# bfloat16/latent-diffusion-speech

Hardware: AMD Instinct MI355X
Metric: mel_frames_per_sec (higher is better)
Workload: dtype f32; 1 GPU; configs[1]: batch=16x512-frame utterances per GPU, 50-step dpm-solver, unet1d denoiser, 80-ch mel; pipeline=sampler, utterances_per_gpu=16, frames=512, nfe=50, method=dpm-solver, parallelism=batch-shard x1

## Files before the change

### latent-diffusion-speech_amd/csrc/kernels.h

```cpp
#pragma once
#include <hip/hip_runtime.h>
#include <stddef.h>
#include <stdint.h>

#include <atomic>
#include <string>

namespace lds {

enum { ACT_NONE = 0, ACT_LRELU = 2 };
enum { EPI_NONE = 0, EPI_GEGLU = 1, EPI_TANH = 2, EPI_GELU = 3, EPI_SWISH = 4, EPI_GLU = 5 };

struct ConvArgs {
    const float* x1; const float* x2;
    int C1, C2;
    int Tsrc;
    int Tin;
    long long xb1, xb2;
    const float* w;
    int Mp, Co, Ci, KT, stride, dil, pad, ups;
    int act_in; float slope;
    const float* bias;
    const float* bias_bc;
    const float* res;
// ... 19 lines not shown

struct ConvDownArgs {
    const float* x; const float* w; const float* bias; float* out;
    int Ci, Co, K, stride, pad, L, To, B;
    float slope;
    int tile;
    const int* vlen_in; const int* vlen;
};
hipError_t launch_conv_down(const ConvDownArgs& a, hipStream_t s);
const char* conv_down_last_config();
hipError_t launch_vae_head(const float* y, const float* noise, float* out, float* z, int B, int C, int T, int only_mean, hipStream_t s,
                           const int* tlen = nullptr);

struct VocPairArgs {
    const float* x; float* out;
    const float* w1; const float* b1; int Mp1;
    const float* w2; const float* b2; int Mp2;
    int C, KT, dil, B, T;
    int accum; float out_div; float slope;
    const int* vlen;
};
bool voc_pair_applies(int C, int KT, int dil);
hipError_t launch_voc_pair(const VocPairArgs& a, hipStream_t s);
const char* voc_pair_last_config();

size_t packed_conv_elems(int Co, int Ci, int K, int* Mp_out);

struct DmaConvArgs {
    const float* x1; const float* x2;
    int C1, C2, Tsrc;
    const float* w;
    const float* bias;
    int Mp, Co, Ci, KT, stride, pad, ups;
    const float* res;
    int epi;
    float* out;
    int out_plain;
    int plain_from; float* out2;
    int vt_D;
    float2* lnpart_out;
    float2* gnpart_out;
    const float2* ln_part; int ln_np; float ln_eps; const float* ln_c1; const float* ln_c2;
    const float2* gnf_part; int gnf_groups; float gnf_eps; const float* gnf_cg; const float* gnf_c2;
    int Cout, To, B;
    int voc;
    int dil;
    int xpad, opad;
    float act_slope;
    float* out_act;
    const float* acc_in;
    float out_div;
    int ph_log2, ph_tpad, ph_Tout, ph_Cout;
    int out_f32;
    float acc_scale;
    int tile_batch;
    const int* lens; int lvl_in, lvl_out;
    const int* vlen;
    int ksplit;
    float* kpart; unsigned* kcount;
    long long kpart_cap; int kcount_cap;
    unsigned ord_m[3], ord_s;
};
struct DmaMagic { unsigned m, s; };
inline DmaMagic dma_magic(unsigned d) {
    unsigned s = 0;
    while ((1ull << s) < d) ++s;
    return DmaMagic{(unsigned)((1ull << (31 + s)) / d + 1), s};
}
__host__ __device__ inline unsigned dma_magic_div(unsigned n, unsigned m, unsigned s) {
    return (unsigned)(((unsigned long long)(n << 1) * m) >> 32) >> s;
}
struct DmaTile { int mb, nb, b, ksp; };
inline DmaTile dma_tile_of(int id, int total, int nMb, int nN, int S, const unsigned* ord_m, unsigned ord_s) {
    const int xcd = id & 7, slot = id >> 3, per = total >> 3, rem = total & 7;
    const unsigned L = (unsigned)(xcd * per + (xcd < rem ? xcd : rem) + slot);
    const unsigned tb = dma_magic_div(L, ord_m[0], ord_s & 255);
    const unsigned by = dma_magic_div(tb, ord_m[1], (ord_s >> 8) & 255);
    const unsigned b = dma_magic_div(by, ord_m[2], (ord_s >> 16) & 255);
    return DmaTile{(int)(L - tb * nMb), (int)(tb - by * nN), (int)b, (int)(by - b * S)};
}
hipError_t launch_conv_dma(const DmaConvArgs& a, int cfg, hipStream_t s);
hipError_t launch_conv_dma_pair(const DmaConvArgs& a3, const DmaConvArgs& a1, hipStream_t s);
bool conv_dma_pair_applies(const DmaConvArgs& a3, const DmaConvArgs& a1);
const char* conv_dma_last_config();

hipError_t launch_conv_bf3(const DmaConvArgs& a, int cfg, int nprod, int fmt, hipStream_t s);
hipError_t launch_conv_bf3_pair(const DmaConvArgs& a3, const DmaConvArgs& a1, int fmt, hipStream_t s);
bool conv_bf3_pair_applies(const DmaConvArgs& a3, const DmaConvArgs& a1);
const char* conv_bf3_last_config();
void conv_bf3_set_debug_rule(int r);
hipError_t launch_to_k8b3(const float* in, void* out, int B, int C, int T, int Ctot, int c_off, hipStream_t s, int fmt = 0, const int* lens = nullptr);
hipError_t launch_from_k8b3(const void* in, float* out, int B, int C, int T, hipStream_t s, int fmt = 0);
hipError_t launch_gn_stream_bf3(const void* x1, const void* x2, int C1, int C2, int T, int groups, float eps, const float* gamma,
                                const float* beta, const float* scale_shift, int ss_stride, int ss_off, int silu, const float2* gp1,
                                const float2* gp2, void* y, int B, hipStream_t s, int fmt = 0, const int* lens = nullptr, int lvl = 0);
hipError_t launch_gn_partials_bf3(const void* x, int C, int T, float2* gp, int B, hipStream_t s, int fmt = 0);
hipError_t launch_resample_k8b3(const void* in, void* out, int B, int C, int Tin, int Tout, hipStream_t s, int fmt = 0, const int* lens = nullptr, int lvl_in = 0, int lvl_out = 0);

hipError_t launch_to_k4p(const float* in, float* out, int B, int C, int T, int Ctot, int c_off, hipStream_t s, const int* lens = nullptr);
hipError_t launch_from_k4p(const float* in, float* out, int B, int C, int T, hipStream_t s);
hipError_t launch_from_k4p_pad(const float* in, float* out, int B, int C, int T, int pad, hipStream_t s);
hipError_t launch_plain_to_vt(const float* in, float* out, int B, int C, int T, int D, hipStream_t s);
hipError_t launch_gn_stream(const float* x1, const float* x2, int C1, int C2, int T, int groups, float eps,
                            const float* gamma, const float* beta, const float* scale_shift, int ss_stride, int ss_off,
                            int silu, const float2* gp1, const float2* gp2, float* y, int B, hipStream_t s, const int* lens = nullptr, int lvl = 0);
hipError_t launch_gn_partials(const float* x, int C, int T, float2* gp, int B, hipStream_t s);
hipError_t launch_to_k4p_act(const float* in, float* raw, float* act, float slope, int B, int C, int T, int pad, hipStream_t s, const int* vlen = nullptr);
hipError_t launch_k4p_zero_pads(float* x, int B, int C, int T, int pad, hipStream_t s);
hipError_t launch_resample_k4p(const float* in, float* out, int B, int C, int Tin, int Tout, hipStream_t s, const int* lens = nullptr, int lvl_in = 0, int lvl_out = 0);
hipError_t launch_attention_k4p(const float* qk, const float* vt, float* out, int B, int C, int T, int heads, hipStream_t s, int tile_batch = 0,
                                const int* lens = nullptr, int lvl = 0);
hipError_t launch_attention_k4p_f16math(const float* qk, const float* vt, float* out, int B, int C, int T, int heads, hipStream_t s, int tile_batch = 0, const int* lens = nullptr);
hipError_t launch_attention_k4p_out_bf3(const float* qk, const float* vt, void* out, int B, int C, int T, int heads, hipStream_t s, int fmt = 0, int tile_batch = 0,
                                        const int* lens = nullptr, int lvl = 0);

hipError_t launch_logmel(const float* audio, const int* slen, long long L, int Fmax, const double* basis, const float* filtT, int n_mels,
                         float* logspec, float* pmax, float* out, int out_k4p, int B, hipStream_t s);
hipError_t launch_whisper_pos(float* x, const float* posk, int n_ctx, float2* lnpart, const int* lens, int B, int C, int T, hipStream_t s);
hipError_t launch_whisper_ln_post(const float* x, const float2* lnpart, const float* gamma, const float* beta, float eps, float* out, const int* lens,
                                  int B, int C, int T, hipStream_t s, int lvl = 1);

hipError_t launch_hubert_conv0(const float* audio, const int* slen, long long L, int pad, const float* w0, const float* gamma, const float* beta, float eps,
                               const int* nlen, int N0, int C, float2* part, float2* stat, float* out, int B, hipStream_t s);
hipError_t launch_hubert_posconv(const float* x, const float* wp, const float* bias, float* out, const int* nlen, int B, int C, int T, int K, int groups,
                                 hipStream_t s);
hipError_t launch_hubert_ln(const float* x, const float* gamma, const float* beta, float eps, float* out, const int* nlen, int B, int C, int T, hipStream_t s);
hipError_t launch_hubert_store_frames(const float* x, float* out, const int* nlen, int B, int C, int T, hipStream_t s);

hipError_t launch_w2v_conv0(const float* audio, const int* slen, long long L, const float* w0, const float* bias, const float* gamma, const float* beta,
                            float eps, const int* nlen, int N0, int C, float* out, int B, hipStream_t s);
hipError_t launch_w2v_ln_act(const float* x, const float* gamma, const float* beta, float eps, float* out, float2* part, const int* nlen, int B, int C, int T,
                             hipStream_t s);
hipError_t launch_w2v_lnpart(const float* x, float2* part, const int* nlen, int B, int C, int T, hipStream_t s);

constexpr int kW2vbertRelStride = 80;
hipError_t launch_w2vbert_fbank(const float* audio, const int* slen, long long L, int Nmax, int Rmax, const double* basis, const float* filtT, int n_mels,
                                int stride, float mel_floor, float* logspec, double2* stat, float* out, int B, hipStream_t s);
hipError_t launch_w2vbert_feats_k4p(const float* feats, float* out, float2* part, const int* vlen, int B, int C, int T, hipStream_t s);
hipError_t launch_w2vbert_relpos(const float* qk, const float* E, float* relp, const int* qlen, int B, int C, int T, int heads, int NR, hipStream_t s);
hipError_t launch_attention_k4p_rel(const float* qk, const float* vt, const float* relp, float* out, int B, int C, int T, int heads, const int* qlens,
                                    const int* klens, int left, int right, hipStream_t s);
hipError_t launch_w2vbert_dwconv(const float* x, const float* wp, const float* gamma, const float* beta, float eps, float* out, const int* vlen,
                                 const int* nlen, int B, int C, int T, int K, hipStream_t s);

hipError_t launch_wavlm_gate(const float* x, const float* w, const float* bias, const float* cst, float* gate, const int* nlen, int B, int C, int T, int heads,
                             hipStream_t s);
hipError_t launch_wavlm_wave_norm(const float* audio, const int* slen, long long L, double2* stat, float* out, int B, hipStream_t s);
hipError_t launch_attention_k4p_bias(const float* qk, const float* vt, const float* gate, const float* toep, float* out, int B, int C, int T, int heads,
                                     const int* lens, int n_ctx, hipStream_t s);

enum { IN_PLAIN = 0, IN_SILU = 1, IN_SINUSOID = 2 };
hipError_t launch_small_linear(const float* W, const float* bias, const float* in, int in_stride, int in_mode,
                               const float* freqs, float* out, int out_stride, int out_silu, int M, int K, int B, hipStream_t s);

enum {
    EW_X0 = 1,
    EW_AXPBY = 2,
    EW_DPM2 = 3,
    EW_UNIPC_PRED = 4,
    EW_UNIPC_CORR = 5,
    EW_UNIPC_CORR1 = 6,
    EW_DDPM = 7,
    EW_DDIM = 8,
    EW_PLMS_PRED = 9,
    EW_LIN4 = 10,
    EW_COPY = 11
};
hipError_t launch_ew(int op, float* out, const float* a, const float* b, const float* c, const float* d,
                     float c0, float c1, float c2, float c3, float c4, long long n, hipStream_t s);
hipError_t launch_dpm_step(float* x, const float* eps, float* m0, const float* m1, float sigma, float alpha, int second, float c4, float c5, float c6,
                           float c7, long long n, hipStream_t s);
hipError_t launch_fill(float* p, float v, long long n, hipStream_t s);
hipError_t launch_touch_lines(const float* p, long long bytes, hipStream_t s);
struct FloatList64 { float f[64]; };
hipError_t launch_set_list(float* dst, const float* host, int n, hipStream_t s);
hipError_t launch_transpose(const float* in, float* out, int B, int R, int C, float scale, hipStream_t s);
hipError_t launch_gather_rows(const float* table, const int64_t* idx, int idx_off, float* out, int B, int C,
                              int nrows, hipStream_t s);
hipError_t launch_resample_frames(const float* in, float* out, int B, int Tin, int Tout, int C, float step, hipStream_t s);
hipError_t launch_resample_nearest(const float* in, float* out, int B, int C, int Tin, int Tout, hipStream_t s);


bool prof_attach_events(hipEvent_t* start, hipEvent_t* stop);
int set_error(int code, const char* fmt, ...);

struct ProfScope {
    bool on;
    hipStream_t s;
    int idx = -1;
    bool attached = false;
    ProfScope(hipStream_t st, const char* name, double flops, double bytes, bool attachable = false);
    ~ProfScope();
    void rename(const std::string& n);
};

inline hipError_t ensure_max_dynamic_lds(const void* kern, std::atomic<unsigned long long>& done) {
    int dev = 0;
    hipError_t e = hipGetDevice(&dev);
    if (e != hipSuccess) return e;
    const unsigned long long bit = 1ull << (dev & 63);
    if (done.load(std::memory_order_acquire) & bit) return hipSuccess;
    e = hipFuncSetAttribute(kern, hipFuncAttributeMaxDynamicSharedMemorySize, 160 * 1024);
    if (e == hipSuccess) done.fetch_or(bit, std::memory_order_release);
    return e;
}

}
```

### latent-diffusion-speech_amd/csrc/misc.hip

```cpp
#include "kernels.h"
#include "../../include/lds.h"

#include <math.h>

namespace lds {

template <int BT>
__global__ void __launch_bounds__(256) small_linear_kernel(const float* __restrict__ W, const float* __restrict__ bias,
                                                           const float* __restrict__ in, int in_stride, int in_mode,
                                                           const float* __restrict__ freqs, float* __restrict__ out,
                                                           int out_stride, int out_silu, int M, int K, int B) {
    const int lane = threadIdx.x & 63;
    const int m = blockIdx.x * 4 + (threadIdx.x >> 6);
    if (m >= M) return;
    const float* wr = W + (long long)m * K;
    for (int b0 = 0; b0 < B; b0 += BT) {
        float acc[BT];
#pragma unroll
        for (int i = 0; i < BT; ++i) acc[i] = 0.f;
        for (int k = lane * 4; k < K; k += 256) {
            const float4 w4 = *reinterpret_cast<const float4*>(wr + k);
            const float wv[4] = {w4.x, w4.y, w4.z, w4.w};
#pragma unroll
            for (int i = 0; i < BT; ++i) {
                if (b0 + i < B) {
#pragma unroll
                    for (int e = 0; e < 4; ++e) {
                        float v;
                        if (in_mode == IN_SINUSOID) {
                            const int half = K >> 1, kk = k + e;
                            const float arg = in[(long long)(b0 + i) * in_stride] * freqs[kk < half ? kk : kk - half];
                            v = (kk < half) ? cosf(arg) : sinf(arg);
                        } else {
                            v = in[(long long)(b0 + i) * in_stride + k + e];
                            if (in_mode == IN_SILU) v = v / (1.0f + expf(-v));
                        }
                        acc[i] = fmaf(wv[e], v, acc[i]);
                    }
                }
            }
        }
#pragma unroll
        for (int i = 0; i < BT; ++i) {
            float v = acc[i];
#pragma unroll
            for (int o = 32; o > 0; o >>= 1) v += __shfl_xor(v, o, 64);
            if (lane == 0 && b0 + i < B) {
                v += bias ? bias[m] : 0.f;
                if (out_silu) v = v / (1.0f + expf(-v));
                out[(long long)(b0 + i) * out_stride + m] = v;
            }
        }
    }
}

hipError_t launch_small_linear(const float* W, const float* bias, const float* in, int in_stride, int in_mode,
                               const float* freqs, float* out, int out_stride, int out_silu, int M, int K, int B, hipStream_t s) {
    if (K % 4) return hipErrorInvalidValue;
    ProfScope ps(s, "small_linear", 2.0 * M * (double)K * B, 4.0 * M * (double)K);
    hipLaunchKernelGGL(small_linear_kernel<16>, dim3((M + 3) / 4), dim3(256), 0, s, W, bias, in, in_stride, in_mode, freqs, out,
                       out_stride, out_silu, M, K, B);
    return hipGetLastError();
}

__global__ void __launch_bounds__(256) ew_kernel(int op, float* __restrict__ out, const float* __restrict__ a,
                                                 const float* __restrict__ b, const float* __restrict__ c,
                                                 const float* __restrict__ d, float c0, float c1, float c2, float c3, float c4,
                                                 long long n) {
    for (long long i = (long long)blockIdx.x * 256 + threadIdx.x; i < n; i += (long long)gridDim.x * 256) {
        float r;
        switch (op) {
            case EW_X0: r = (a[i] - c0 * b[i]) / c1; break;
            case EW_AXPBY: r = c0 * a[i] - c1 * b[i]; break;
            case EW_DPM2: { const float bi = b[i]; r = c0 * a[i] - c1 * bi - c2 * (c3 * (bi - c[i])); } break;
            case EW_UNIPC_PRED: r = a[i] - c0 * (c1 * ((c[i] - b[i]) / c2)); break;
            case EW_UNIPC_CORR: { const float bi = b[i]; r = a[i] - c0 * (c1 * ((d[i] - bi) / c2) + c3 * (c[i] - bi)); } break;
            case EW_UNIPC_CORR1: r = a[i] - c0 * (c3 * (c[i] - b[i])); break;
            case EW_DDPM: {
                const float ai = a[i];
                float x0 = c0 * ai - c1 * b[i];
                x0 = fminf(fmaxf(x0, -1.0f), 1.0f);
                r = (c2 * x0 + c3 * ai) + c4 * c[i];
            } break;
            case EW_DDIM: r = c0 * (a[i] / c1 + c2 * b[i]); break;
            case EW_PLMS_PRED: { const float ai = a[i]; r = ai + c0 * (c1 * ai - c2 * b[i]); } break;
            case EW_LIN4: {
                float v = c0 * a[i];
                if (b) v += c1 * b[i];
                if (c) v += c2 * c[i];
                if (d) v += c3 * d[i];
                r = v / c4;
            } break;
            default: r = a[i]; break;
        }
        out[i] = r;
    }
}

hipError_t launch_ew(int op, float* out, const float* a, const float* b, const float* c, const float* d, float c0, float c1,
                     float c2, float c3, float c4, long long n, hipStream_t s) {
    long long blocks = (n + 255) / 256;
    if (blocks > 4096) blocks = 4096;
    ProfScope ps(s, "ew", 0.0, 4.0 * 3.0 * (double)n);
    hipLaunchKernelGGL(ew_kernel, dim3((unsigned)blocks), dim3(256), 0, s, op, out, a, b, c, d, c0, c1, c2, c3, c4, n);
    return hipGetLastError();
}

__global__ void __launch_bounds__(256) dpm_step_kernel(float* __restrict__ x, const float* __restrict__ eps, float* __restrict__ m0, const float* __restrict__ m1,
                                                       float sigma, float alpha, int second, float c4, float c5, float c6, float c7, long long n) {
    for (long long i = (long long)blockIdx.x * 256 + threadIdx.x; i < n; i += (long long)gridDim.x * 256) {
        const float xi = x[i];
        const float bi = (xi - sigma * eps[i]) / alpha;
        m0[i] = bi;
        x[i] = second ? c4 * xi - c5 * bi - c6 * (c7 * (bi - m1[i])) : c4 * xi - c5 * bi;
    }
}
hipError_t launch_dpm_step(float* x, const float* eps, float* m0, const float* m1, float sigma, float alpha, int second, float c4, float c5, float c6,
                           float c7, long long n, hipStream_t s) {
    long long blocks = (n + 255) / 256;
    if (blocks > 4096) blocks = 4096;
    ProfScope ps(s, "ew", 0.0, 4.0 * (second ? 5.0 : 4.0) * (double)n);
    hipLaunchKernelGGL(dpm_step_kernel, dim3((unsigned)blocks), dim3(256), 0, s, x, eps, m0, m1, sigma, alpha, second, c4, c5, c6, c7, n);
    return hipGetLastError();
}

__global__ void __launch_bounds__(256) fill_kernel(float* p, float v, long long n) {
    for (long long i = (long long)blockIdx.x * 256 + threadIdx.x; i < n; i += (long long)gridDim.x * 256) p[i] = v;
}
__global__ void __launch_bounds__(256) touch_lines_kernel(const float* p, long long n_lines, float* sink) {
    const long long i = (long long)blockIdx.x * 256 + threadIdx.x;
    float v = 0.f;
    if (i < n_lines) v = p[i * 16];
    if (v == 1.2345678e-30f && sink) sink[0] = v;
}
hipError_t launch_touch_lines(const float* p, long long bytes, hipStream_t s) {
    const long long n_lines = bytes / 64;
    if (n_lines <= 0) return hipSuccess;
    hipLaunchKernelGGL(touch_lines_kernel, dim3((unsigned)((n_lines + 255) / 256)), dim3(256), 0, s, p, n_lines, (float*)nullptr);
    return hipGetLastError();
}

hipError_t launch_fill(float* p, float v, long long n, hipStream_t s) {
    long long blocks = (n + 255) / 256;
    if (blocks > 4096) blocks = 4096;
    ProfScope ps(s, "fill", 0.0, 4.0 * (double)n);
    hipLaunchKernelGGL(fill_kernel, dim3((unsigned)blocks), dim3(256), 0, s, p, v, n);
    return hipGetLastError();
}

__global__ void __launch_bounds__(64) set_list_kernel(float* __restrict__ dst, FloatList64 v, int n) {
    if ((int)threadIdx.x < n) dst[threadIdx.x] = v.f[threadIdx.x];
}
hipError_t launch_set_list(float* dst, const float* host, int n, hipStream_t s) {
    if (n < 0 || n > 64) return hipErrorInvalidValue;
    FloatList64 v;
    for (int i = 0; i < 64; ++i) v.f[i] = i < n ? host[i] : 0.f;
    hipLaunchKernelGGL(set_list_kernel, dim3(1), dim3(64), 0, s, dst, v, n);
    return hipGetLastError();
}

__global__ void __launch_bounds__(256) transpose_kernel(const float* __restrict__ in, float* __restrict__ out, int R, int C, float scale) {
    __shared__ float tile[32][33];
    const int b = blockIdx.z;
    const int r0 = blockIdx.y * 32, c0 = blockIdx.x * 32;
    const int tx = threadIdx.x & 31, ty = threadIdx.x >> 5;
    const float* ib = in + (long long)b * R * C;
    float* ob = out + (long long)b * R * C;
#pragma unroll
    for (int i = 0; i < 4; ++i) {
        const int r = r0 + ty + i * 8, cc = c0 + tx;
        tile[ty + i * 8][tx] = (r < R && cc < C) ? ib[(long long)r * C + cc] : 0.f;
    }
    __syncthreads();
#pragma unroll
    for (int i = 0; i < 4; ++i) {
        const int cc = c0 + ty + i * 8, r = r0 + tx;
        if (cc < C && r < R) ob[(long long)cc * R + r] = (scale == 1.0f) ? tile[tx][ty + i * 8] : tile[tx][ty + i * 8] / scale;
    }
}
hipError_t launch_transpose(const float* in, float* out, int B, int R, int C, float scale, hipStream_t s) {
    hipLaunchKernelGGL(transpose_kernel, dim3((C + 31) / 32, (R + 31) / 32, B), dim3(256), 0, s, in, out, R, C, scale);
    return hipGetLastError();
}

__global__ void gather_rows_kernel(const float* __restrict__ table, const int64_t* __restrict__ idx, int idx_off,
                                   float* __restrict__ out, int C, int nrows) {
    const int b = blockIdx.x;
    const long long r = idx[b] + idx_off;
    const bool ok = r >= 0 && r < nrows;
    for (int cc = threadIdx.x; cc < C; cc += blockDim.x) out[(long long)b * C + cc] = ok ? table[r * C + cc] : __builtin_nanf("");
}
hipError_t launch_gather_rows(const float* table, const int64_t* idx, int idx_off, float* out, int B, int C, int nrows, hipStream_t s) {
    hipLaunchKernelGGL(gather_rows_kernel, dim3(B), dim3(256), 0, s, table, idx, idx_off, out, C, nrows);
    return hipGetLastError();
}

__global__ void resample_frames_kernel(const float* __restrict__ in, float* __restrict__ out, int Tin, int Tout, int C, float step) {
    const int i = blockIdx.x, b = blockIdx.y;
    int src = (int)floorf((float)i * step);
    if (src > Tin - 1) src = Tin - 1;
    const float* ib = in + ((long long)b * Tin + src) * C;
    float* ob = out + ((long long)b * Tout + i) * C;
    for (int cc = threadIdx.x; cc < C; cc += blockDim.x) ob[cc] = ib[cc];
}
hipError_t launch_resample_frames(const float* in, float* out, int B, int Tin, int Tout, int C, float step, hipStream_t s) {
    if (B <= 0 || Tin <= 0 || Tout <= 0 || C <= 0) return hipErrorInvalidValue;
    hipLaunchKernelGGL(resample_frames_kernel, dim3(Tout, B), dim3(256), 0, s, in, out, Tin, Tout, C, step);
    return hipGetLastError();
}

__global__ void __launch_bounds__(256) resample_nearest_kernel(const float* __restrict__ in, float* __restrict__ out, int Tin, int Tout, long long rows) {
    const float sc = (float)Tin / (float)Tout;
    for (long long i = (long long)blockIdx.x * 256 + threadIdx.x; i < rows * Tout; i += (long long)gridDim.x * 256) {
        const long long r = i / Tout;
        const int t = (int)(i - r * Tout);
        int src = (int)floorf((float)t * sc);
        if (src > Tin - 1) src = Tin - 1;
        out[i] = in[r * Tin + src];
    }
}
hipError_t launch_resample_nearest(const float* in, float* out, int B, int C, int Tin, int Tout, hipStream_t s) {
    const long long rows = (long long)B * C;
    long long blocks = (rows * Tout + 255) / 256;
    if (blocks > 4096) blocks = 4096;
    hipLaunchKernelGGL(resample_nearest_kernel, dim3((unsigned)blocks), dim3(256), 0, s, in, out, Tin, Tout, rows);
    return hipGetLastError();
}

}

namespace lds {

__global__ void __launch_bounds__(256) q_sample_rows_kernel(float* __restrict__ out, const float* __restrict__ x0, const float* __restrict__ noise,
                                                            const long long* __restrict__ t, const float* __restrict__ sa, const float* __restrict__ s1,
                                                            int n_steps, float* __restrict__ tf, long long n) {
#pragma clang fp contract(off)
    const int b = blockIdx.y;
    long long tb = t[b];
    tb = tb < 0 ? 0 : tb >= n_steps ? n_steps - 1 : tb;
    const float c0 = sa[tb], c1 = s1[tb];
    if (tf && blockIdx.x == 0 && threadIdx.x == 0) tf[b] = (float)tb;
    const long long o = (long long)b * n;
    for (long long i = (long long)blockIdx.x * 256 + threadIdx.x; i < n; i += (long long)gridDim.x * 256)
        out[o + i] = __fadd_rn(__fmul_rn(c0, x0[o + i]), __fmul_rn(c1, noise[o + i]));
}

constexpr int LR_SLICE = 4096;

static __device__ __forceinline__ double block_sum_256(double v, double* red) {
    red[threadIdx.x] = v;
    __syncthreads();
#pragma unroll
    for (int o = 128; o > 0; o >>= 1) {
        if ((int)threadIdx.x < o) red[threadIdx.x] += red[threadIdx.x + o];
        __syncthreads();
    }
    return red[0];
}

__global__ void __launch_bounds__(256) loss_partial_kernel(const float* __restrict__ a, const float* __restrict__ b, long long n, int l2,
                                                           double* __restrict__ part) {
    __shared__ double red[256];
    const long long base = (long long)blockIdx.x * LR_SLICE;
    double s = 0.0;
#pragma unroll
    for (int e = 0; e < LR_SLICE / 256; ++e) {
        const long long i = base + e * 256 + threadIdx.x;
        if (i < n) {
            const float d = __fsub_rn(a[i], b[i]);
            s += l2 ? (double)__fmul_rn(d, d) : (double)fabsf(d);
        }
    }
    s = block_sum_256(s, red);
    if (threadIdx.x == 0) part[blockIdx.x] = s;
}

__global__ void __launch_bounds__(256) loss_finish_kernel(const double* __restrict__ part, int nblk, long long n, float* __restrict__ out) {
    __shared__ double red[256];
    double s = 0.0;
    for (int i = threadIdx.x; i < nblk; i += 256) s += part[i];
    s = block_sum_256(s, red);
    if (threadIdx.x == 0) out[0] = (float)(s / (double)n);
}

}

namespace {
constexpr long long kLossMaxN = 1LL << 40;
long long loss_blocks(long long n) { return (n + lds::LR_SLICE - 1) / lds::LR_SLICE; }
}

extern "C" int lds_q_sample_rows(float* out, const float* x0, const float* noise, const int64_t* t, const float* sqrt_ac, const float* sqrt_1m_ac, int n_steps,
                                 float* t_f32, int B, int64_t n, void* stream) {
    if (!out || !x0 || !noise || !t || !sqrt_ac || !sqrt_1m_ac) return lds::set_error(LDS_EINVAL, "lds_q_sample_rows: null pointer");
    if (n_steps < 1 || B < 1 || B > 65535 || n < 1) return lds::set_error(LDS_EINVAL, "lds_q_sample_rows: bad argument");
    long long blocks = (n + 255) / 256;
    if (blocks > 1024) blocks = 1024;
    hipStream_t s = (hipStream_t)stream;
    lds::ProfScope ps(s, "ew", 0.0, 4.0 * 3.0 * (double)n * B);
    hipLaunchKernelGGL(lds::q_sample_rows_kernel, dim3((unsigned)blocks, B), dim3(256), 0, s, out, x0, noise, reinterpret_cast<const long long*>(t), sqrt_ac,
                       sqrt_1m_ac, n_steps, t_f32, (long long)n);
    const hipError_t e = hipGetLastError();
    return e == hipSuccess ? LDS_OK : lds::set_error(LDS_EHIP, "lds_q_sample_rows: %s", hipGetErrorString(e));
}

extern "C" int lds_loss_reduce_workspace_bytes(int64_t n, size_t* out) {
    if (!out || n < 1 || n > kLossMaxN) return lds::set_error(LDS_EINVAL, "lds_loss_reduce_workspace_bytes: bad argument");
    *out = (size_t)loss_blocks(n) * sizeof(double);
    return LDS_OK;
}

extern "C" int lds_loss_reduce(const float* a, const float* b, int64_t n, int loss_type, float* out, void* ws, size_t ws_bytes, void* stream) {
    if (!a || !b || !out || !ws) return lds::set_error(LDS_EINVAL, "lds_loss_reduce: null pointer");
    if (n < 1 || n > kLossMaxN) return lds::set_error(LDS_EINVAL, "lds_loss_reduce: n %lld outside 1 .. %lld", (long long)n, kLossMaxN);
    if (loss_type != 1 && loss_type != 2) return lds::set_error(LDS_EINVAL, "lds_loss_reduce: loss_type %d (1 = l1, 2 = l2)", loss_type);
    const long long nblk = loss_blocks(n);
    if (ws_bytes < (size_t)nblk * sizeof(double)) return lds::set_error(LDS_ENOMEM, "lds_loss_reduce: workspace %zu < %zu bytes", ws_bytes, (size_t)nblk * sizeof(double));
    if (((uintptr_t)ws & 7) != 0) return lds::set_error(LDS_EINVAL, "lds_loss_reduce: the workspace must be 8-byte aligned");
    hipStream_t s = (hipStream_t)stream;
    lds::ProfScope ps(s, "loss_reduce", 3.0 * (double)n, 8.0 * (double)n);
    hipLaunchKernelGGL(lds::loss_partial_kernel, dim3((unsigned)nblk), dim3(256), 0, s, a, b, (long long)n, loss_type == 2 ? 1 : 0, (double*)ws);
    hipError_t e = hipGetLastError();
    if (e == hipSuccess) {
        hipLaunchKernelGGL(lds::loss_finish_kernel, dim3(1), dim3(256), 0, s, (const double*)ws, (int)nblk, (long long)n, out);
        e = hipGetLastError();
    }
    return e == hipSuccess ? LDS_OK : lds::set_error(LDS_EHIP, "lds_loss_reduce: %s", hipGetErrorString(e));
}
```

### latent-diffusion-speech_amd/lds/native.py

```python
import ctypes as C
import os

import numpy as np

_HERE = os.path.dirname(os.path.abspath(__file__))
LIB_PATH = os.path.join(_HERE, "liblds.so")
_lib = None

METHODS = {"dpm-solver": 1, "unipc": 2, "ddpm": 3, "ddim": 4, "pndm": 5}
TABLE_STRIDE = 16


class UNetCfg(C.Structure):
    _fields_ = [("out_dims", C.c_int), ("n_hidden", C.c_int), ("n_layers", C.c_int), ("n_heads", C.c_int),
                ("norm_groups", C.c_int), ("n_blocks", C.c_int), ("block_out_channels", C.c_int * 8)]


class VocoderCfg(C.Structure):
    _fields_ = [("inter_channels", C.c_int), ("upsample_initial_channel", C.c_int), ("n_ups", C.c_int),
                ("upsample_rates", C.c_int * 8), ("upsample_kernel_sizes", C.c_int * 8), ("resblock", C.c_int),
                ("n_kernels", C.c_int), ("resblock_kernel_sizes", C.c_int * 4), ("n_dil", C.c_int),
                ("resblock_dilation_sizes", (C.c_int * 4) * 4)]


# ... 56 lines not shown
lds_transpose                    i:ppiiifp
lds_gather_rows                  i:pppiiip
lds_resample_frames              i:ppiiiifp
lds_axpby                        i:pppffqp
lds_q_sample_rows                i:ppppppipiqp
lds_loss_reduce_workspace_bytes  i:qp
lds_loss_reduce                  i:ppqippzp
lds_stft_mel_workspace_bytes     i:iiiiqp
lds_stft_mel                     i:ppppiiiiiifippziqp
lds_vocoder_create               i:pipppp
lds_vocoder_destroy              v:p
lds_vocoder_workspace_bytes      i:piip
lds_vocoder_forward              i:ppppziip
lds_vocoder_forward_ragged       i:pppppziip
lds_vae_encoder_create           i:pipppp
lds_vae_encoder_destroy          v:p
lds_vae_encoder_workspace_bytes  i:piqp
lds_vae_encoder_forward          i:pppppipziqp
lds_vae_encoder_forward_ragged   i:ppppppipziqp
lds_whisper_create               i:pippppp
lds_whisper_destroy              v:p
lds_whisper_workspace_bytes      i:piqp
lds_whisper_logmel               i:pppppziqp
lds_whisper_encode_mel           i:pppppziip
lds_whisper_encode               i:pppppziqp
lds_hubert_create                i:pipppp
lds_hubert_destroy               v:p
lds_hubert_workspace_bytes       i:piqip
lds_hubert_features              i:pppppziqip
lds_hubert_encode                i:ppppiipziqip
lds_w2v_create                   i:pipppp
lds_w2v_destroy                  v:p
lds_w2v_workspace_bytes          i:piqp
lds_w2v_features                 i:pppppziqp
lds_w2v_encode                   i:pppppziqp
lds_wavlm_create                 i:pipppp
lds_wavlm_destroy                v:p
lds_wavlm_workspace_bytes        i:piqp
lds_wavlm_features               i:ppppipziqp
lds_wavlm_encode                 i:ppppiipziqp
lds_w2vbert_create               i:pipppp
lds_w2vbert_destroy              v:p
lds_w2vbert_workspace_bytes      i:piqp
lds_w2vbert_fbank                i:pppppziqp
lds_w2vbert_encode_features      i:pppppziip
lds_w2vbert_encode               i:pppppziqp
lds_lm_create                    i:pipppp
lds_lm_destroy                   v:p
lds_lm_workspace_bytes           i:piiip
lds_lm_encode                    i:pppppppziip
lds_lm_generate                  i:pppiiiiifffpppppzp
lds_lm_workspace_bytes_opts      i:piiiip
lds_lm_generate_opts             i:pppiiippppppzp
lds_lm_workspace_bytes_prompt    i:piiiip
lds_lm_generate_prompt           i:pppiiipppipppppzp
lds_lm_score_workspace_bytes     i:piiip
lds_lm_score                     i:pppiipppippppppzp
lds_llama_create                 i:pipppp
lds_llama_destroy                v:p
lds_llama_workspace_bytes        i:piiip
lds_llama_generate               i:pppiiippppppzp
lds_llama_beam_workspace_bytes   i:piiiip
lds_llama_generate_beam          i:pppiiippppzp
lds_llama_score_workspace_bytes  i:piip
lds_llama_score                  i:ppppiippppppzp
lds_kmeans_workspace_bytes       i:qiip
lds_kmeans_prepare               i:piipp
lds_kmeans_assign                i:pqppiipppzp
lds_kmeans_assign_ragged         i:piipqppiipppzp
lds_kmeans_update                i:ppqpppiippzp
lds_kmeans_seed                  i:pqiiqppppzp
lds_knn_prepare                  i:pqipp
lds_knn_workspace_bytes          i:qqiip
lds_knn_search                   i:pqppqiipppzp
lds_knn_retrieve                 i:pqppqiifppppzp
lds_knn_retrieve_ragged          i:piipppqiifppppzp
lds_ivf_workspace_bytes          i:qqiiiip
lds_ivf_search                   i:pqppqiippippppqipppzp
lds_ivf_retrieve                 i:pqppqiippippppqifppppzp
lds_ivf_retrieve_ragged          i:piipppqiippippppqifppppzp
lds_resample                     i:ppppiiiiqqp
lds_resample_ragged              i:ppppppiiiiqqp
lds_frame_rms                    i:ppqiiiqp
lds_volume_extract               i:ppqpqp
lds_volume_mask                  i:ppqifp
lds_resample_frames_ragged       i:ppppiiiip
lds_overlap_assemble             i:pqppipqpqp
lds_prof_enable                  i:i
lds_prof_summary                 i:pz
lds_unet_set_gemm_mode           i:pi
lds_unet_get_gemm_mode           i:p
lds_unet_set_latency_mode        i:pi
lds_unet_get_latency_mode        i:p
"""
_TEST = """
lds_test_conv                    i:ppip
lds_test_dconv                   i:pppip
lds_bench_dconv                  i:ppiippzp
lds_test_gn_apply                i:ppiiiifpppipip
lds_bench_gn_stream              i:iiiiipp
lds_test_gn_chain_k4p            i:pppppfiippiiiiip
lds_test_ln_chain_k4p            i:pppppfppiiiip
lds_test_attention_k4p           i:ppiiiip
lds_test_conv_transpose          i:ppppiiiiiiifp
lds_test_voc_step                i:pppppiiiiipfppip
lds_test_dconv_bf3               i:pppiip
lds_bench_dconv_bf3              i:ppiiippzp
lds_test_k8b3_roundtrip          i:ppiiip
lds_test_gn_apply_bf3            i:ppiiiifpppipip
lds_test_dconv_split             i:pppiiip
lds_bench_dconv_split            i:ppiiiippzp
lds_test_split_roundtrip         i:ppiiiip
lds_test_gn_apply_split          i:ppiiiifpppipiip
lds_debug_set_split_rule         i:i
lds_test_attention_f16math       i:ppiiiip
lds_test_attention_latency       i:ppiiiiip
lds_test_attention_ragged        i:pppiiiiiip
lds_debug_set_gn_fold            i:i
lds_debug_set_voc_pair           i:i
lds_debug_set_touch_weights      i:i
lds_test_voc_pair                i:pppppiiiipfppip
lds_test_gn_fold_k4p             i:pppppfippppiiiiiiip
lds_bench_dconv_alt              i:ppiipipp
lds_debug_fill_u32               i:pzup
lds_debug_trace                  i:i
lds_debug_trace_count            i:
lds_debug_trace_get              i:ipzpp
lds_debug_unet_plan              i:piipz
lds_test_gn_fold_split           i:pppppfippppiiiiiiiiip
lds_test_cluster_join            i:ppppiiiiiiippppzp
lds_test_lm_sample               i:piiiifffppipp
lds_test_conv_down               i:pppiiiiiifippzp
lds_test_conv_down_ragged        i:pppiiiiiifppippzp
lds_test_lm_beam_step            i:piiiiiifiippppppppppppppppp
lds_test_llama_beam_step         i:piiiiiifiiipppppppppppppppppppp
lds_test_llama_beam_attn         i:pppppiiiiiiiipp
lds_test_llama_generate_beam_poll i:pppiiippppzpi
lds_test_dconv_pair              i:pppppppiiiiiipiiipppzp
lds_test_dconv_ex                i:pppipzp
lds_test_dma_magic_div           i:uup
lds_test_dma_tile_order          i:iiiip
lds_test_tap_k4p                 i:pz
lds_test_voc_ups                 i:pppiiiiiipppppzp
lds_test_w2v_conv0               i:ppppppfpiiqp
lds_test_w2v_ln_act              i:ppppfppiiip
lds_test_w2vbert_fbank           i:pppiqp
lds_test_w2vbert_attention       i:pppppiiiiiip
lds_test_w2vbert_dwconv          i:ppppfpppiiiip
lds_test_wavlm_attention         i:pppppiiiiip
lds_test_wavlm_buckets           i:iiip
lds_test_stft_dft                i:pppiiiippiqp
lds_test_knn_search              i:pqppqiiiipppzp
lds_test_ivf_search              i:pqppqiippippppqiipppzp
"""
SIGNATURES = dict(ln.split() for ln in (_PUBLIC + _TEST).splitlines() if ln)
EXPORTS = [ln.split()[0] for ln in _PUBLIC.splitlines() if ln]
TEST_EXPORTS = [ln.split()[0] for ln in _TEST.splitlines() if ln]


def lib():
    global _lib
    if _lib is None:
        if not os.path.exists(LIB_PATH):
            raise RuntimeError(f"{LIB_PATH} is missing: build it with `make -C latent-diffusion-speech_amd/csrc` "
                               "(there is no CPU fallback for the hot path)")
        L = C.CDLL(LIB_PATH)
        for n in EXPORTS + TEST_EXPORTS:
            ret, _, args = SIGNATURES[n].partition(":")
            fn = getattr(L, n)
            fn.restype, fn.argtypes = _RETURN[ret], [_KIND[k] for k in args]
        _lib = L
    return _lib


def check(rc):
    if rc != 0:
        raise RuntimeError(f"liblds error {rc}: {lib().lds_last_error().decode()}")


def _stream():
    import torch
    return C.c_void_p(torch.cuda.current_stream().cuda_stream)


def _dev(t, dtype=None):
    import torch
    if not t.is_cuda:
        raise RuntimeError("liblds needs tensors on a HIP device (no CPU fallback for the hot path)")
    if not t.is_contiguous():
        raise RuntimeError("liblds needs contiguous tensors")
    if dtype is not None and t.dtype != dtype:
        raise RuntimeError(f"expected {dtype}, got {t.dtype}")
    return C.c_void_p(t.data_ptr())


def _host_tensor_table(state):
    names, ptrs, numel, keep = [], [], [], []
    for k, v in state.items():
        a = v.detach().cpu().numpy() if hasattr(v, "detach") else np.asarray(v)
        a = np.ascontiguousarray(a, dtype=np.float32)
        keep.append(a)
        names.append(k.encode())
        ptrs.append(a.ctypes.data)
        numel.append(a.size)
    n = len(names)
    return (n, (C.c_char_p * n)(*names), (C.c_void_p * n)(*ptrs), (C.c_int64 * n)(*numel), keep)


class Workspace:

    def __init__(self):
        self.bufs = {}

    def get(self, nbytes, device):
        import torch
        key = (str(device), int(torch.cuda.current_stream(device).cuda_stream))
        buf = self.bufs.get(key)
        if buf is None or buf.numel() < nbytes:
            buf = torch.empty(int(nbytes), dtype=torch.uint8, device=device)
            self.bufs[key] = buf
        return buf


def _dev_or_null(t, dtype=None):
    return None if t is None else _dev(t, dtype)


def _host(a):
    return None if a is None else a.ctypes.data


def _bytes(entry, *args):
    nb = C.c_size_t()
    check(getattr(lib(), entry)(*args, C.byref(nb)))
    return nb.value


def _host_lengths(lengths, B, lo, hi, max_B=None, what=""):
    if max_B is not None and B > max_B:
        raise ValueError(f"a ragged {what} batch holds at most {max_B} clips (got {B})")
    a = np.ascontiguousarray(np.asarray(lengths.cpu() if hasattr(lengths, "cpu") else lengths).reshape(-1), dtype=np.int32)
    if a.shape != (B,) or a.min() < lo or a.max() > hi:
        raise ValueError(f"lengths must be {B} integers in {lo} .. {hi}")
    return a


def _dense_or_ragged(name, *lengths):
    if lengths[0] is None:
        return getattr(lib(), name), ()
    return getattr(lib(), name + "_ragged"), tuple(a.ctypes.data for a in lengths)


class _Handle:
    KIND = None

    def _create(self, *args):
        self.h, self.ws = C.c_void_p(), Workspace()
        check(getattr(lib(), f"lds_{self.KIND}_create")(*args, C.byref(self.h)))

    def _create_weights(self, cfg, state, *more):
        n, names, ptrs, numel, keep = _host_tensor_table(state)
        self._create(C.byref(cfg), n, names, ptrs, numel, *more)

    def __del__(self):
        if getattr(self, "h", None) and _lib is not None:
            getattr(_lib, f"lds_{self.KIND}_destroy")(self.h)
            self.h = None

    def _workspace(self, entry, device, *dims):
        return self.ws.get(_bytes(entry, self.h, *dims), device)


class UNet(_Handle):
    KIND = "unet"

    def __init__(self, cfg, state):
        c = UNetCfg()
        c.out_dims, c.n_hidden = cfg["out_channels"], cfg["cond_channels"]
        c.n_layers, c.n_heads, c.norm_groups = cfg["layers_per_block"], cfg["heads"], cfg["groups"]
        boc = cfg["block_out_channels"]
        c.n_blocks = len(boc)
        for i, v in enumerate(boc):
            c.block_out_channels[i] = v
        self._create_weights(c, state)
        self.M, self.H = c.out_dims, c.n_hidden

    def set_gemm_mode(self, mode):
        m = {"f32": 0, "split_bf16": 1, "split_f16": 2}.get(mode, mode)
        check(lib().lds_unet_set_gemm_mode(self.h, int(m)))

    def gemm_mode(self):
        return int(lib().lds_unet_get_gemm_mode(self.h))

    def set_latency_mode(self, on):
        check(lib().lds_unet_set_latency_mode(self.h, 1 if on else 0))

    def latency_mode(self):
        return int(lib().lds_unet_get_latency_mode(self.h))

    @staticmethod
    def _lengths(lengths, B, T):
        return _host_lengths(lengths, B, 1, T)

    def workspace_tensor(self, B, T, device, sampler=False):
        return self._workspace("lds_sampler_workspace_bytes" if sampler else "lds_unet_workspace_bytes", device, B, T)

# ... 918 lines not shown
    M, D = pool.shape
    if x.dim() != 2 or x.shape[1] != D:
        raise ValueError(f"ivf_search: x {list(x.shape)} against a pool {[M, D]}")
    N = x.shape[0]
    ws = _ivf_ws_for(ws, N, M, D, k, ivf, nprobe, x.device)
    idx = torch.empty(N, k, dtype=torch.int32, device=x.device)
    score = torch.empty(N, k, dtype=torch.float32, device=x.device)
    head = (_dev(x, torch.float32), N, _dev(pool, torch.float32), _dev(h, torch.float32), M, D, int(k), *_ivf_args(ivf, nprobe))
    tail = (_dev(idx), _dev(score), _dev(ws), ws.numel(), _stream())
    if slab_rows is None:
        check(lib().lds_ivf_search(*head, *tail))
    else:
        check(lib().lds_test_ivf_search(*head, int(slab_rows), *tail))
    return idx, score


def ivf_retrieve(x, pool, h, k, ratio, ivf, nprobe, lengths=None, ws=None):
    import torch
    M, D = pool.shape
    if x.shape[-1] != D or x.dim() != (3 if lengths is not None else 2):
        raise ValueError(f"ivf_retrieve: x {list(x.shape)} against a pool {[M, D]}")
    N = x.numel() // D
    ws = _ivf_ws_for(ws, N, M, D, k, ivf, nprobe, x.device)
    y = torch.empty_like(x)
    idx = torch.empty(*x.shape[:-1], k, dtype=torch.int32, device=x.device)
    dist = torch.empty(*x.shape[:-1], k, dtype=torch.float32, device=x.device)
    ln = None if lengths is None else _host_lengths(lengths, x.shape[0], 0, x.shape[1], max_B=64, what="retrieval")
    fn, ln_at = _dense_or_ragged("lds_ivf_retrieve", ln)
    rows = (N,) if ln is None else (x.shape[0], x.shape[1], *ln_at)
    check(fn(_dev(x, torch.float32), *rows, _dev(pool, torch.float32), _dev(h, torch.float32), M, D, int(k), *_ivf_args(ivf, nprobe), float(ratio), _dev(y),
             _dev(idx), _dev(dist), _dev(ws), ws.numel(), _stream()))
    return y, idx, dist


_resample_tables = {}


def resample_tables(orig_freq, new_freq, lowpass_filter_width=6, rolloff=0.99):
    key = (orig_freq, new_freq, lowpass_filter_width, float(rolloff))
    t = _resample_tables.get(key)
    if t is None:
        from . import arch
        O, N, taps, bankT, first = arch.resample_bank(*key)
        t = _resample_tables[key] = dict(O=O, N=N, taps=taps, bankT=bankT, first=first, dev={})
    return t


def resample_out_length(length, O, N):
    return -((-int(length) * N) // O)


def resample(x, tables, lengths=None):
    import torch
    if not x.is_cuda:
        raise RuntimeError("liblds needs tensors on a HIP device (no CPU fallback for the hot path)")
    B, L = x.shape
    O, N = tables["O"], tables["N"]
    dev = tables["dev"].get(str(x.device))
    if dev is None:
        dev = tables["dev"][str(x.device)] = (torch.from_numpy(tables["bankT"]).to(x.device), torch.from_numpy(tables["first"]).to(x.device))
    ln = None if lengths is None else _host_lengths(lengths, B, 0, L, max_B=64, what="resampler")
    M = resample_out_length(L if ln is None else max(int(ln.max()), 1), O, N)
    y = torch.empty((B, M), dtype=torch.float32, device=x.device)
    tail = (_dev(dev[0], torch.float32), _dev(dev[1], torch.int32), O, N, tables["taps"], B, L, M, _stream())
    if ln is None:
        check(lib().lds_resample(_dev(x, torch.float32), _dev(y), *tail))
        return y
    new = np.zeros(B, dtype=np.int64)
    check(lib().lds_resample_ragged(_dev(x, torch.float32), _host(ln), _dev(y), _host(new), *tail))
    return y, torch.from_numpy(new)


def _wave_1d(x, what):
    import torch
    if not torch.is_tensor(x) or not x.is_cuda:
        raise RuntimeError(f"{what} needs the audio as a tensor on a HIP device (no CPU fallback)")
    if x.dim() != 1 or x.numel() < 1:
        raise ValueError(f"{what}: a mono 1-D waveform with at least one sample is needed, got shape {list(x.shape)}")
    return x.float().contiguous()


def frame_rms_length(L, frame_length, hop_length):
    return 1 + (int(L) + 2 * (frame_length // 2) - frame_length) // hop_length


def frame_rms(x, frame_length, hop_length, pad_mode="constant"):
    import torch
    if pad_mode not in ("constant", "reflect"):
        raise ValueError(f"frame_rms: pad_mode {pad_mode!r} ('constant' or 'reflect')")
    x = _wave_1d(x, "frame_rms")
    n = frame_rms_length(x.numel(), frame_length, hop_length)
    out = torch.empty(max(n, 0), dtype=torch.float32, device=x.device)
    check(lib().lds_frame_rms(_dev(x, torch.float32), _dev(out), x.numel(), int(frame_length), int(hop_length), int(pad_mode == "reflect"), n, _stream()))
    return out


def volume_extract(x, hop):
    import torch
    x = _wave_1d(x, "volume_extract")
    hop = float(hop)
    if not hop >= 1.0:
        raise ValueError(f"volume_extract: hop {hop} must be at least 1")
    n = int(x.numel() // hop) + 1
    out = torch.empty(n, dtype=torch.float32, device=x.device)
    h = C.c_double(hop)
    check(lib().lds_volume_extract(_dev(x, torch.float32), _dev(out), x.numel(), C.addressof(h), n, _stream()))
    return out


def volume_mask(volume, factor, threshold):
    import torch
    if not torch.is_tensor(volume) or not volume.is_cuda:
        raise RuntimeError("volume_mask needs the volume as a tensor on a HIP device (no CPU fallback)")
    v = volume.reshape(-1).float().contiguous()
    out = torch.empty(v.numel() * int(factor), dtype=torch.float32, device=v.device)
    check(lib().lds_volume_mask(_dev(v, torch.float32), _dev(out), v.numel(), int(factor), float(np.float32(threshold)), _stream()))
    return out


def resample_frames_ragged(x, tin, tout):
    import torch
    B, T, Cc = x.shape
    ti = _host_lengths(tin, B, 1, T, max_B=64, what="frame alignment")
    to = _host_lengths(tout, B, 0, 2 ** 31 - 1)
    n_out = max(int(to.max()), 1)
    out = torch.empty(B, n_out, Cc, dtype=torch.float32, device=x.device)
    check(lib().lds_resample_frames_ragged(_dev(x, torch.float32), _host(ti), _host(to), _dev(out), B, T, n_out, Cc, _stream()))
    return out


def overlap_table(offset, start, length):
    tab = np.ascontiguousarray(np.stack([np.asarray(a, dtype=np.int64).reshape(-1) for a in (offset, start, length)]))
    if tab.shape[1] < 1:
        raise ValueError("overlap_assemble: no segment")
    return tab


def overlap_assemble(segs, offset, start, length, mask=None):
    import torch
    tab = overlap_table(offset, start, length)
    S = tab.shape[1]
    N = int(tab[1, -1] + tab[2, -1])
    if not torch.is_tensor(segs) or not segs.is_cuda or (mask is not None and not mask.is_cuda):
        raise RuntimeError("liblds needs tensors on a HIP device (no CPU fallback for the hot path)")
    m = None if mask is None else mask.reshape(-1)
    dtab = torch.from_numpy(tab).to(segs.device)
    out = torch.empty(min(max(N, 0), 1 << 33), dtype=torch.float32, device=segs.device)
    rc = lib().lds_overlap_assemble(_dev(segs, torch.float32) if segs.numel() else None, segs.numel(), _host(tab), _dev(dtab, torch.int64), S,
                                    _dev_or_null(m, torch.float32), 0 if m is None else m.numel(), _dev(out) if N > 0 else None, N, _stream())
    if rc == -1:
        raise ValueError(lib().lds_last_error().decode())
    check(rc)
    return out
```

Measured before the change: 25140 mel-frames/s.

## Add LDS-staged small_linear kernel with multi-row waves and weight prefetch

```diff
diff --git a/latent-diffusion-speech_amd/csrc/kernels.h b/latent-diffusion-speech_amd/csrc/kernels.h
--- a/latent-diffusion-speech_amd/csrc/kernels.h
+++ b/latent-diffusion-speech_amd/csrc/kernels.h
@@ -195,6 +195,8 @@
 enum { IN_PLAIN = 0, IN_SILU = 1, IN_SINUSOID = 2 };
 hipError_t launch_small_linear(const float* W, const float* bias, const float* in, int in_stride, int in_mode,
                                const float* freqs, float* out, int out_stride, int out_silu, int M, int K, int B, hipStream_t s);
+hipError_t launch_small_linear_path(const float* W, const float* bias, const float* in, int in_stride, int in_mode, const float* freqs, float* out,
+                                    int out_stride, int out_silu, int M, int K, int B, int path, hipStream_t s);
 
 enum {
     EW_X0 = 1,
diff --git a/latent-diffusion-speech_amd/csrc/misc.hip b/latent-diffusion-speech_amd/csrc/misc.hip
--- a/latent-diffusion-speech_amd/csrc/misc.hip
+++ b/latent-diffusion-speech_amd/csrc/misc.hip
@@ -1,5 +1,6 @@
 #include "kernels.h"
 #include "../../include/lds.h"
+#include "../../include/lds_test.h"
 
 #include <math.h>
 
@@ -54,13 +55,205 @@
     }
 }
 
+constexpr int kSlCols = 32;
+constexpr int kSlMaxK = 1024;
+constexpr int kSlThreads = 512;
+constexpr int kSlWaves = kSlThreads / 64;
+
+template <int V, int U>
+static __device__ __forceinline__ void sl_stage_plain(float* sf, const float* __restrict__ in, int in_stride, int silu, int b0, int B, int ncp, int K) {
+    const int KV = K / V, total = ncp * KV;
+    for (int i0 = threadIdx.x; i0 < total; i0 += kSlThreads * U) {
+        float t[U][V];
+#pragma unroll
+        for (int u = 0; u < U; ++u) {
+            const int idx = i0 + u * kSlThreads;
+#pragma unroll
+            for (int e = 0; e < V; ++e) t[u][e] = 0.f;
+            if (idx < total) {
+                const int bb = idx / KV, kk = (idx - bb * KV) * V;
+                if (b0 + bb < B) {
+                    const float* src = in + (long long)(b0 + bb) * in_stride + kk;
+                    if constexpr (V == 4) {
+                        const float4 q = *reinterpret_cast<const float4*>(src);
+                        t[u][0] = q.x; t[u][1] = q.y; t[u][2] = q.z; t[u][3] = q.w;
+                    } else {
+                        t[u][0] = src[0];
+                    }
+                }
+            }
+        }
+#pragma unroll
+        for (int u = 0; u < U; ++u) {
+            const int idx = i0 + u * kSlThreads;
+            if (idx < total) {
+#pragma unroll
+                for (int e = 0; e < V; ++e) {
+                    float v = t[u][e];
+                    if (silu) v = v / (1.0f + expf(-v));
+                    sf[idx * V + e] = v;
+                }
+            }
+        }
+    }
+}
+
+template <int NJ>
+__global__ void __launch_bounds__(kSlThreads) small_linear_staged_kernel(const float* __restrict__ W, const float* __restrict__ bias,
+                                                                  const float* __restrict__ in, int in_stride, int in_mode, int in_vec,
+                                                                  const float* __restrict__ freqs, float* __restrict__ out,
+                                                                  int out_stride, int out_silu, int M, int K, int B) {
+    extern __shared__ float4 sl_in[];
+    float* sf = reinterpret_cast<float*>(sl_in);
+    const int lane = threadIdx.x & 63;
+    const int K4 = K >> 2;
+    const int gw = blockIdx.x * kSlWaves + __builtin_amdgcn_readfirstlane(threadIdx.x >> 6), nw = gridDim.x * kSlWaves;
+    const int npair = (M + 1) >> 1;
+    auto load_w = [&](float4 (&w)[2][NJ], int pr) {
+#pragma unroll
+        for (int r = 0; r < 2; ++r) {
+            const int m = (2 * pr + r < M) ? 2 * pr + r : M - 1;
+            const float* wr = W + (long long)m * K;
+#pragma unroll
+            for (int j = 0; j < NJ; ++j) {
+                const int k = lane * 4 + 256 * j;
+                w[r][j] = (k < K) ? *reinterpret_cast<const float4*>(wr + k) : float4{0.f, 0.f, 0.f, 0.f};
+            }
+        }
+    };
+    for (int b0 = 0; b0 < B; b0 += kSlCols) {
+        const int nc = (B - b0 < kSlCols) ? B - b0 : kSlCols;
+        const int ng = (nc + 7) >> 3, ncp = ng * 8;
+        if (b0) __syncthreads();
+        if (in_mode == IN_SINUSOID) {
+            const int half = K >> 1;
+            for (int idx = threadIdx.x; idx < ncp * K; idx += kSlThreads) {
+                const int bb = idx / K, kk = idx - bb * K;
+                float v = 0.f;
+                if (b0 + bb < B) {
+                    const float arg = in[(long long)(b0 + bb) * in_stride] * freqs[kk < half ? kk : kk - half];
+                    v = (kk < half) ? cosf(arg) : sinf(arg);
+                }
+                sf[idx] = v;
+            }
+        } else if (in_vec) {
+            sl_stage_plain<4, 8>(sf, in, in_stride, in_mode == IN_SILU, b0, B, ncp, K);
+        } else {
+            sl_stage_plain<1, 8>(sf, in, in_stride, in_mode == IN_SILU, b0, B, ncp, K);
+        }
+        __syncthreads();
+        float4 wc[2][NJ];
+        if (gw < npair) load_w(wc, gw);
+        for (int pr = gw; pr < npair; pr += nw) {
+            float4 wn[2][NJ];
+            load_w(wn, (pr + nw < npair) ? pr + nw : pr);
+            float acc[2][kSlCols];
+#pragma unroll
+            for (int r = 0; r < 2; ++r)
+#pragma unroll
+                for (int i = 0; i < kSlCols; ++i) acc[r][i] = 0.f;
+#pragma unroll
+            for (int j = 0; j < NJ; ++j) {
+                if (lane * 4 + 256 * j < K) {
+#pragma unroll
+                    for (int g = 0; g < kSlCols / 8; ++g) {
+                        if (g < ng) {
+#pragma unroll
+                            for (int i = g * 8; i < g * 8 + 8; ++i) {
+                                const float4 v4 = sl_in[i * K4 + 64 * j + lane];
+                                const float vv[4] = {v4.x, v4.y, v4.z, v4.w};
+#pragma unroll
+                                for (int r = 0; r < 2; ++r) {
+                                    const float wv[4] = {wc[r][j].x, wc[r][j].y, wc[r][j].z, wc[r][j].w};
+#pragma unroll
+                                    for (int e = 0; e < 4; ++e) acc[r][i] = fmaf(wv[e], vv[e], acc[r][i]);
+                                }
+                            }
+                        }
+                    }
+                }
+            }
+            float red[2 * kSlCols];
+#pragma unroll
+            for (int r = 0; r < 2; ++r)
+#pragma unroll
+                for (int i = 0; i < kSlCols; ++i) red[kSlCols * r + i] = acc[r][i];
+#pragma unroll
+            for (int o = 32; o > 0; o >>= 1) {
+                const bool up = (lane & o) != 0;
+#pragma unroll
+                for (int q = 0; q < o; ++q) {
+                    const float send = up ? red[q] : red[q + o], keep = up ? red[q + o] : red[q];
+                    red[q] = keep + __shfl_xor(send, o, 64);
+                }
+            }
+            const float res = red[0];
+            const int m = 2 * pr + (lane >> 5), col = b0 + (lane & 31);
+            if (m < M && col < B) {
+                float v = res;
+                v += bias ? bias[m] : 0.f;
+                if (out_silu) v = v / (1.0f + expf(-v));
+                out[(long long)col * out_stride + m] = v;
+            }
+#pragma unroll
+            for (int r = 0; r < 2; ++r)
+#pragma unroll
+                for (int j = 0; j < NJ; ++j) wc[r][j] = wn[r][j];
+        }
+    }
+}
+
+static int small_linear_cus() {
+    static std::atomic<int> cus[64];
+    int dev = 0;
+    if (hipGetDevice(&dev) != hipSuccess) return 0;
+    std::atomic<int>& c = cus[dev & 63];
+    int n = c.load(std::memory_order_relaxed);
+    if (n == 0) {
+        if (hipDeviceGetAttribute(&n, hipDeviceAttributeMultiprocessorCount, dev) != hipSuccess || n <= 0) return 0;
+        c.store(n, std::memory_order_relaxed);
+    }
+    return n;
+}
+
+template <int NJ>
+static hipError_t launch_small_linear_staged(const float* W, const float* bias, const float* in, int in_stride, int in_mode, const float* freqs,
+                                             float* out, int out_stride, int out_silu, int M, int K, int B, hipStream_t s) {
+    static std::atomic<unsigned long long> lds_raised{0};
+    const void* kern = reinterpret_cast<const void*>(&small_linear_staged_kernel<NJ>);
+    hipError_t e = ensure_max_dynamic_lds(kern, lds_raised);
+    if (e != hipSuccess) return e;
+    const int cus = small_linear_cus();
+    if (cus <= 0) return hipErrorInvalidDevice;
+    const int wgs = ((M + 1) / 2 + kSlWaves - 1) / kSlWaves;
+    const int in_vec = in_mode != IN_SINUSOID && in_stride % 4 == 0 && ((uintptr_t)in & 15) == 0;
+    hipLaunchKernelGGL(small_linear_staged_kernel<NJ>, dim3(wgs < cus ? wgs : cus), dim3(kSlThreads), (size_t)kSlCols * K * sizeof(float), s, W, bias, in,
+                       in_stride, in_mode, in_vec, freqs, out, out_stride, out_silu, M, K, B);
+    return hipGetLastError();
+}
+
+hipError_t launch_small_linear_path(const float* W, const float* bias, const float* in, int in_stride, int in_mode, const float* freqs, float* out,
+                                    int out_stride, int out_silu, int M, int K, int B, int path, hipStream_t s) {
+    if (K % 4 || K < 4 || M < 1 || B < 1 || path < 0 || path > 2) return hipErrorInvalidValue;
+    const bool can = K <= kSlMaxK;
+    if (path == 2 && !can) return hipErrorInvalidValue;
+    ProfScope ps(s, "small_linear", 2.0 * M * (double)K * B, 4.0 * M * (double)K);
+    if (path == 2 || (path == 0 && can && B > 1)) {
+        switch ((K + 255) / 256) {
+            case 1: return launch_small_linear_staged<1>(W, bias, in, in_stride, in_mode, freqs, out, out_stride, out_silu, M, K, B, s);
+            case 2: return launch_small_linear_staged<2>(W, bias, in, in_stride, in_mode, freqs, out, out_stride, out_silu, M, K, B, s);
+            case 3: return launch_small_linear_staged<3>(W, bias, in, in_stride, in_mode, freqs, out, out_stride, out_silu, M, K, B, s);
+            default: return launch_small_linear_staged<4>(W, bias, in, in_stride, in_mode, freqs, out, out_stride, out_silu, M, K, B, s);
+        }
+    }
+    hipLaunchKernelGGL(small_linear_kernel<16>, dim3((M + 3) / 4), dim3(256), 0, s, W, bias, in, in_stride, in_mode, freqs, out,
+                       out_stride, out_silu, M, K, B);
+    return hipGetLastError();
+}
+
 hipError_t launch_small_linear(const float* W, const float* bias, const float* in, int in_stride, int in_mode,
                                const float* freqs, float* out, int out_stride, int out_silu, int M, int K, int B, hipStream_t s) {
-    if (K % 4) return hipErrorInvalidValue;
-    ProfScope ps(s, "small_linear", 2.0 * M * (double)K * B, 4.0 * M * (double)K);
-    hipLaunchKernelGGL(small_linear_kernel<16>, dim3((M + 3) / 4), dim3(256), 0, s, W, bias, in, in_stride, in_mode, freqs, out,
-                       out_stride, out_silu, M, K, B);
-    return hipGetLastError();
+    return launch_small_linear_path(W, bias, in, in_stride, in_mode, freqs, out, out_stride, out_silu, M, K, B, 0, s);
 }
 
 __global__ void __launch_bounds__(256) ew_kernel(int op, float* __restrict__ out, const float* __restrict__ a,
@@ -327,3 +520,44 @@
     }
     return e == hipSuccess ? LDS_OK : lds::set_error(LDS_EHIP, "lds_loss_reduce: %s", hipGetErrorString(e));
 }
+
+static int small_linear_entry(const char* who, const float* W, const float* bias, const float* in, int in_stride, int in_mode, const float* freqs, float* out,
+                              int out_stride, int out_silu, int M, int K, int B, int path, int iters, float* ms_out, hipStream_t s) {
+    if (!W || !in || !out || (in_mode == lds::IN_SINUSOID && !freqs)) return lds::set_error(LDS_EINVAL, "%s: null pointer", who);
+    if (in_mode < lds::IN_PLAIN || in_mode > lds::IN_SINUSOID || M < 1 || K < 4 || K % 4 || B < 1 || out_stride < M || path < 0 || path > 2 || iters < 1)
+        return lds::set_error(LDS_EINVAL, "%s: bad argument", who);
+    if (in_mode != lds::IN_SINUSOID && in_stride < K) return lds::set_error(LDS_EINVAL, "%s: in_stride %d < K %d", who, in_stride, K);
+    if (path == 2 && K > lds::kSlMaxK) return lds::set_error(LDS_EINVAL, "%s: the staged kernel takes K <= %d (got %d)", who, lds::kSlMaxK, K);
+    hipEvent_t e0 = nullptr, e1 = nullptr;
+    hipError_t e = hipSuccess;
+    if (ms_out) {
+        if ((e = hipEventCreate(&e0)) == hipSuccess) e = hipEventCreate(&e1);
+        for (int w = 0; w < 3 && e == hipSuccess; ++w)
+            e = lds::launch_small_linear_path(W, bias, in, in_stride, in_mode, freqs, out, out_stride, out_silu, M, K, B, path, s);
+        if (e == hipSuccess) e = hipEventRecord(e0, s);
+    }
+    for (int i = 0; i < iters && e == hipSuccess; ++i)
+        e = lds::launch_small_linear_path(W, bias, in, in_stride, in_mode, freqs, out, out_stride, out_silu, M, K, B, path, s);
+    if (ms_out && e == hipSuccess) e = hipEventRecord(e1, s);
+    if (e == hipSuccess) e = hipStreamSynchronize(s);
+    if (ms_out && e == hipSuccess) {
+        float ms = 0.f;
+        if ((e = hipEventElapsedTime(&ms, e0, e1)) == hipSuccess) *ms_out = ms / (float)iters;
+    }
+    if (e0) (void)hipEventDestroy(e0);
+    if (e1) (void)hipEventDestroy(e1);
+    return e == hipSuccess ? LDS_OK : lds::set_error(LDS_EHIP, "%s: %s", who, hipGetErrorString(e));
+}
+
+extern "C" int lds_test_small_linear(const float* W, const float* bias, const float* in, int in_stride, int in_mode, const float* freqs, float* out,
+                                     int out_stride, int out_silu, int M, int K, int B, int path, void* stream) {
+    return small_linear_entry("lds_test_small_linear", W, bias, in, in_stride, in_mode, freqs, out, out_stride, out_silu, M, K, B, path, 1, nullptr,
+                              (hipStream_t)stream);
+}
+
+extern "C" int lds_bench_small_linear(const float* W, const float* bias, const float* in, int in_stride, int in_mode, const float* freqs, float* out,
+                                      int out_stride, int out_silu, int M, int K, int B, int path, int iters, float* ms_out, void* stream) {
+    if (!ms_out) return lds::set_error(LDS_EINVAL, "lds_bench_small_linear: null pointer");
+    return small_linear_entry("lds_bench_small_linear", W, bias, in, in_stride, in_mode, freqs, out, out_stride, out_silu, M, K, B, path, iters, ms_out,
+                              (hipStream_t)stream);
+}
diff --git a/latent-diffusion-speech_amd/lds/native.py b/latent-diffusion-speech_amd/lds/native.py
--- a/latent-diffusion-speech_amd/lds/native.py
+++ b/latent-diffusion-speech_amd/lds/native.py
@@ -232,6 +232,8 @@
 lds_test_stft_dft                i:pppiiiippiqp
 lds_test_knn_search              i:pqppqiiiipppzp
 lds_test_ivf_search              i:pqppqiippippppqiipppzp
+lds_test_small_linear            i:pppiippiiiiiip
+lds_bench_small_linear           i:pppiippiiiiiiipp
 """
 SIGNATURES = dict(ln.split() for ln in (_PUBLIC + _TEST).splitlines() if ln)
 EXPORTS = [ln.split()[0] for ln in _PUBLIC.splitlines() if ln]
@@ -1456,3 +1458,24 @@
         raise ValueError(lib().lds_last_error().decode())
     check(rc)
     return out
+
+
+SMALL_LINEAR_IN = {"plain": 0, "silu": 1, "sinusoid": 2}
+
+
+def small_linear(W, bias, x, in_mode="plain", freqs=None, out_silu=False, path=0, out_stride=None, iters=0):
+    import torch
+    M, K = W.shape
+    B = x.shape[0]
+    mode = SMALL_LINEAR_IN[in_mode]
+    in_stride = 1 if mode == 2 else x.shape[1]
+    stride = M if out_stride is None else int(out_stride)
+    out = torch.full((B, stride), float("nan"), dtype=torch.float32, device=W.device)
+    args = (_dev(W, torch.float32), _dev_or_null(bias, torch.float32), _dev(x, torch.float32), in_stride, mode, _dev_or_null(freqs, torch.float32),
+            _dev(out), stride, int(bool(out_silu)), M, K, B, int(path))
+    if iters > 0:
+        ms = C.c_float(0.0)
+        check(lib().lds_bench_small_linear(*args, int(iters), C.byref(ms), _stream()))
+        return out, float(ms.value)
+    check(lib().lds_test_small_linear(*args, _stream()))
+    return out
```

After: 25200 mel-frames/s, median of 6. About the same (+0.2%).
